# dillonalaird/pysvihmm

Hardware: AMD Instinct MI355X
Metric: obs-state updates/sec (T*K/s) per SVI E-step, K=64 Gaussian HMM (higher is better)
Workload: dtype f64

## Files before the change

include/svihmm_debug.h:

```cpp
#ifndef SVIHMM_DEBUG_H
#define SVIHMM_DEBUG_H

#include "svihmm.h"

#ifdef __cplusplus
extern "C" {
#endif

#define SVIHMM_NKERN 12
#define SVIHMM_PROF_SLOTS 0x40000000
int svihmm_profile_enable(svihmm_ctx* h, int32_t on);
int svihmm_profile_reset(svihmm_ctx* h);
int svihmm_profile_read(svihmm_ctx* h, double ms_out[SVIHMM_NKERN],
                        int64_t count_out[SVIHMM_NKERN]);
const char* svihmm_kernel_name(int32_t slot);
const char* svihmm_last_kernel_name(svihmm_ctx* h, int32_t slot);
#define SVIHMM_NVARIANT 24
enum {
  SVIHMM_VAR_SVI_LOOP = 0,
  SVIHMM_VAR_STATS = 1,
  SVIHMM_VAR_FB = 2,
  SVIHMM_VAR_EMISSION_MT = 3,
  SVIHMM_VAR_PIPELINE = 4,
  SVIHMM_VAR_EMISSION_ORBIT = 5,
  SVIHMM_VAR_CHAIN = 6,
  SVIHMM_VAR_SWEEP_FAMILY = 7,
  SVIHMM_VAR_STATS_CHUNKS = 8,
  SVIHMM_VAR_CENTRING = 9,
  SVIHMM_VAR_STATS_TILING = 10,
  SVIHMM_VAR_ALLREDUCE_COORDS = 11,
  SVIHMM_VAR_STATS_LDS3 = 12,
  SVIHMM_VAR_WIDE_SWEEPS = 13,
  SVIHMM_VAR_WIDE_TRAN_BLOCK = 14,
  SVIHMM_VAR_WIDE_POSTERIOR = 15,
  SVIHMM_VAR_RENORM4 = 16,
  SVIHMM_VAR_MSG_LAYOUT = 17
};
enum {
  SVIHMM_SVI_LOOP_EVENTS = 1,
  SVIHMM_SVI_LOOP_LOSE_CONCURRENCY = 2,
  SVIHMM_SVI_LOOP_STUCK_GATE = 3,
  SVIHMM_SVI_LOOP_NO_ELBO = 9,
  SVIHMM_STATS_DBUF = 2,
  SVIHMM_STATS_PIPELINED = 3,
  SVIHMM_FB_WAVE = 1,
  SVIHMM_FB_LOG_MFMA = 2,
  SVIHMM_FB_SCALED = 3,
  SVIHMM_EMISSION_MT_NT4 = 1,
  SVIHMM_PIPELINE_UNFUSED = 1,
  SVIHMM_PIPELINE_TWO_STREAM = 2,
  SVIHMM_PIPELINE_FUSED_ALL = 3,
  SVIHMM_PIPELINE_FUSED_EMISSION = 5,
  SVIHMM_PIPELINE_F32_OWN = 6,
  SVIHMM_EMISSION_ORBIT_OFF = 1,
  SVIHMM_EMISSION_ORBIT_128 = 2,
  SVIHMM_EMISSION_ORBIT_F64 = 3,
  SVIHMM_EMISSION_ORBIT_BF16_SMALL = 4,
  SVIHMM_EMISSION_ORBIT_64 = 5,
  SVIHMM_EMISSION_ORBIT_GENERIC_EDGES = 6,
  SVIHMM_EMISSION_ORBIT_128_GENERIC_EDGES = 7,
  SVIHMM_EMISSION_ORBIT_BF16_128 = 8,
  SVIHMM_CHAIN_OFF = 1,
  SVIHMM_SWEEP_FAMILY_ONE_TILE = 1,
  SVIHMM_SWEEP_FAMILY_TILES = 2,
  SVIHMM_SWEEP_FAMILY_WAVE_LIN = 3,
  SVIHMM_SWEEP_FAMILY_WAVE_LIN4 = 4,
  SVIHMM_SWEEP_FAMILY_SKIP = 9,
  SVIHMM_CENTRING_OFF = 1,
  SVIHMM_CENTRING_PULL_STARTS = 2,
  SVIHMM_STATS_TILING_FIVE = 1,
  SVIHMM_STATS_TILING_F32_MFMA = 2,
  SVIHMM_STATS_TILING_BF16_SMALL = 3,
  SVIHMM_ALLREDUCE_COORDS_ON = 1,
  SVIHMM_STATS_LDS3_OFF = 1,
  SVIHMM_STATS_LDS3_FLAT = 2,
  SVIHMM_WIDE_SWEEPS_16 = 1,
  SVIHMM_WIDE_SWEEPS_THETA_OLD = 2,
  SVIHMM_WIDE_SWEEPS_THETA_OWN_STEP = 3,
  SVIHMM_WIDE_TRAN_BLOCK_64 = 1,
  SVIHMM_WIDE_POSTERIOR_PASS = 1,
  SVIHMM_WIDE_POSTERIOR_PASS_ALL = 2,
  SVIHMM_RENORM4_OFF = 1,
  SVIHMM_MSG_LAYOUT_ROW_MAJOR = 1
};
int svihmm_set_variant(svihmm_ctx* h, int32_t which, int32_t value);
int svihmm_svi_recoveries(svihmm_ctx* h, int32_t* out);
// ... 9 lines not shown
```

pysvihmm_amd/_lib.py:

```python
import ctypes as C
import os

import numpy as np

_HERE = os.path.dirname(os.path.abspath(__file__))
LIB_PATH = os.path.join(_HERE, "libsvihmm_hip.so")

ABI_VERSION = 3
NKERN = 12
PROF_SLOTS = 0x40000000
MASK_AS_NAN = 1
TRANS_WRAP = 2
USE_HOST_LLIKS = 4
KEEP_LBETA = 8
SVI_KEEP_WINDOW = 16
SVI_MIN_PSEUDOCOUNT = 2.5e-3
LTRAN_LINEAR_MIN = -600.0
NIW_MAX_D = 96
DIAG_MAX_D = 128
MCAT_MAX_D = 128
MCAT_MAX_F = 1024
POISSON_MAX_D = 128
POISSON_MAX_COUNT = (1 << 20) - 1
PGAUSS_MAX_D = 128
PGAUSS_ABSENT = 1e150
LTRAN_F32_MIN = -60.0
F64, F32 = 0, 1
GROW_METHOD = {"auto": 0, "literal": 1, "products": 2}
VARIANT = {
    "svi_loop": 0, "stats": 1, "fb": 2, "emission_mt": 3, "pipeline": 4, "emission_orbit": 5, "chain": 6,
    "sweep_family": 7, "stats_chunks": 8, "centring": 9, "stats_tiling": 10, "allreduce_coords": 11,
    "stats_lds3": 12, "wide_sweeps": 13, "wide_tran_block": 14, "wide_posterior": 15, "renorm4": 16,
    "msg_layout": 17,
}
EMISSION_ORBIT_128 = 2
EMISSION_ORBIT_GENERIC_EDGES = 6
EMISSION_ORBIT_128_GENERIC_EDGES = 7

_lib = None

_c_double_p = C.POINTER(C.c_double)
_c_int64_p = C.POINTER(C.c_int64)
_c_uint8_p = C.POINTER(C.c_uint8)

SIGNATURES = {
    "svihmm_last_error": (C.c_char_p, []),
    "svihmm_abi_version": (C.c_int, []),
    "svihmm_device_count": (C.c_int, [C.POINTER(C.c_int)]),
    "svihmm_create": (C.c_int, [C.c_int, C.POINTER(C.c_void_p)]),
    "svihmm_destroy": (C.c_int, [C.c_void_p]),
    "svihmm_sync": (C.c_int, [C.c_void_p]),
    "svihmm_set_precision": (C.c_int, [C.c_void_p, C.c_int32]),
    "svihmm_get_precision": (C.c_int, [C.c_void_p, C.POINTER(C.c_int32), C.POINTER(C.c_int32)]),
    "svihmm_set_obs": (C.c_int, [C.c_void_p, _c_double_p, C.c_int64, C.c_int32, _c_uint8_p]),
    "svihmm_set_globals": (C.c_int, [C.c_void_p, C.c_int32, _c_double_p, _c_double_p]),
    "svihmm_set_emission_niw": (C.c_int, [C.c_void_p, C.c_int32, C.c_int32, _c_double_p,
                                          _c_double_p, _c_double_p, _c_double_p]),
    "svihmm_set_emission_diag": (C.c_int, [C.c_void_p, C.c_int32, C.c_int32, _c_double_p,
                                           _c_double_p, _c_double_p, _c_double_p]),
    "svihmm_set_lliks": (C.c_int, [C.c_void_p, _c_double_p, C.c_int32, C.c_int32]),
    "svihmm_loglik": (C.c_int, [C.c_void_p, _c_int64_p, C.c_int32, C.c_int32, C.c_uint32,
                                _c_double_p]),
    "svihmm_forward_backward": (C.c_int, [C.c_void_p, _c_int64_p, C.c_int32, C.c_int32,
                                          C.c_uint32, _c_double_p, _c_double_p, _c_double_p,
                                          _c_double_p]),
    "svihmm_packed_size": (C.c_int64, [C.c_int32, C.c_int32]),
    "svihmm_estep_minibatch": (C.c_int, [C.c_void_p, _c_int64_p, C.c_int32, C.c_int32,
                                         C.c_uint32, _c_double_p]),
    "svihmm_read_packed": (C.c_int, [C.c_void_p, _c_double_p]),
    "svihmm_suffstats": (C.c_int, [C.c_void_p, _c_int64_p, C.c_int32, C.c_int32, C.c_uint32,
# ... 159 lines not shown
```

pysvihmm_amd/csrc/host.h:

```cpp
#pragma once
#include <hip/hip_runtime.h>
#include <rccl/rccl.h>

#include <cmath>
#include <cstdint>
#include <cstdio>
#include <cstring>
#include <cstdlib>
#include <string>
#include <type_traits>
#include <vector>

#include "../../include/svihmm.h"
#include "../../include/svihmm_debug.h"
#include "svihmm_common.h"

extern thread_local std::string g_err;
inline int fail(const std::string& m) { g_err = m; return 1; }
#define HIPCK(x)                                                                   \
  do {                                                                             \
    hipError_t e_ = (x);                                                           \
    if (e_ != hipSuccess)                                                          \
      return fail(std::string(#x) + ": " + hipGetErrorString(e_) + " (" __FILE__ \
                  ":" + std::to_string(__LINE__) + ")");                           \
// ... 77 lines not shown
  int eK = 0, eD = 0, Kp = 0, F = 0, Fp = 0;
  Buf theta, theta_orb, fab, niw, cat_table, partc, prior, vlb_aux, gen_z;
  int64_t gen_T = 0;
  double* vlb_host = nullptr;
  int prior_K = 0, prior_D = 0, vlb_host_K = 0;
  void *slack_a = nullptr, *slack_t = nullptr;
  int slack_k = 0;
  void* orb_zero_p = nullptr; size_t orb_zero_n = 0;
  const double* chain_kbef = nullptr; int chain_C = 0, chain_L = 0, chain_T = 0;
  int lb_pending = 0;
  bool orb_valid = false;
  Buf uwb;
  void* uw_zero_p = nullptr;
  bool uw_valid = false;
  Buf uwd;
  void* uwd_zero_p = nullptr; size_t uwd_zero_n = 0;
  bool uwd_valid = false, emd_attr_set[2] = {false, false};
  bool emb_attr_set = false;
  EmisFamily fam = EF_NIW;
  int V = 0;
  Buf mcat_meta;
  int pois_C = 0; Buf pois_logfact; std::vector<double> pois_lf_host;
  Buf pg_origin;
  bool tab_diag = false;
  void* theta_zero_p = nullptr; size_t theta_zero_n = 0;
  int tabD = -1;
  struct PinSlot { void* p = nullptr; size_t cap = 0; hipEvent_t ev = nullptr; bool busy = false; };
  PinSlot pins[6];
  int pin_next = 0;
  struct StartSlot { void* p = nullptr; size_t cap = 0; int used_it = -1; };
  StartSlot svi_starts[8];
  const int64_t* starts_pending = nullptr;
  int starts_pending_n = 0;
  bool starts_sync_call = false, starts_slot_inflight = false;
  void* starts_slot = nullptr; size_t starts_slot_cap = 0;
  int svi_upload_it = -1;
  int* pin_status = nullptr;
  double* mirror = nullptr; size_t mirror_cap = 0;
  bool mirror_valid = false;
  bool status_pending = false;
  bool status_auto = false;
  bool have_emission = false;
  Buf starts, ll, la, lb, q, lse_part, local_lb, logz, part, packed, scratch;
  Buf user_q, user_starts;
  std::vector<int64_t> seq_off;
  Buf seq_off_d, seq_q, seq_work, seq_ord, seq_out;
  bool seq_internal = false;
  bool seq_result = false;
  Buf sub_obs, sub_mask, sub_tab;
  bool seq_subset = false;
  Buf labels, sub_labels;
  bool have_labels = false;
  int32_t label_max = -1; int64_t label_max_row = -1;
  Buf sets, sub_sets;
  bool have_sets = false;
  int32_t sets_K = 0, sets_W = 0;
  Buf dec_tab;
  std::vector<char> dec_host;
  int dec_result = 0;
  int post_kind = 0, post_K = 0, post_fam = -1;
  Buf heldout;
  Buf vit;
  Buf kexp, hx, gx, zfac, llE, m_ll, m_la, m_lb, chain, chain2;
  Buf ll0, a0v, a0e;
  bool lin_mode = false;
  bool q_valid = false;
// ... 162 lines not shown
int ensure_stats(svihmm_ctx* h, int64_t nchunk_total);
int flush_lb(svihmm_ctx* h, hipStream_t stream);
int launch_diag_to_theta(svihmm_ctx* h, int K, int D);
int launch_emission(svihmm_ctx* h, int B, int Lm, uint32_t flags, bool scaled = false, const int64_t* starts_dev = nullptr, double* out = nullptr, double* kexp_out = nullptr, hipStream_t stream = nullptr, size_t min_lds = 0, double* ll0_out = nullptr, bool clamp_labels = true);
int check_labels_fit(const svihmm_ctx* h);
int check_sets_fit(const svihmm_ctx* h);
int check_clamp_fit(const svihmm_ctx* h);
int launch_fb(svihmm_ctx* h, int B, int Lm, int dir0, int ndir, const double* ll = nullptr, double* la = nullptr, double* lb = nullptr);
int launch_fb_fused(svihmm_ctx* h, int B, int Lm, bool want_lb, bool total);
bool emission_row_tile_orbit(const svihmm_ctx* h, int64_t n);
bool step_major_ok(const svihmm_ctx* h, int B, int Lm, uint32_t flags, bool lin);
int launch_fb_lin(svihmm_ctx* h, int B, int Lm, bool total);
int launch_fb_lin_range(svihmm_ctx* h, int b0, int nb, int Lm, hipStream_t stream);
int launch_niw_to_theta(svihmm_ctx* h, int K, int D, double* logdet_out, const SviStepArgs* step = nullptr);
bool step_theta_ok(const svihmm_ctx* h, int K, int D);
int launch_posterior(svihmm_ctx* h, int B, int Lm, bool total);
int launch_scale_ll(svihmm_ctx* h, int B, int Lm);
int launch_scale_ll_f32(svihmm_ctx* h, int B, int Lm);
bool f32_wide_ok(const svihmm_ctx* h, int64_t n);
bool stats_bf16w_shape_ok(const svihmm_ctx* h, int64_t n);
int launch_stats(svihmm_ctx* h, int B, int Lq, int off, int Lm, uint32_t flags);
int launch_stats_finalize(svihmm_ctx* h, int64_t nchunk, hipStream_t stream);
int launch_stats_range(svihmm_ctx* h, int b0, int nb, int Lq, int off, int Lm, uint32_t flags, StatsPlan plan, int64_t chunk_base, hipStream_t stream,
                       const double* qsrc = nullptr, const int64_t* starts_src = nullptr);
int launch_stats_posteriors(svihmm_ctx* h, const double* q, const int64_t* starts_dev, int B, int Lm, uint32_t flags);
int launch_sum_lb(svihmm_ctx* h, int B, hipStream_t stream);
int materialise(svihmm_ctx* h, int b0, int nb);
int prepare_ll(svihmm_ctx* h, const int64_t* starts, int B, int Lm, uint32_t flags, bool need_obs_for_stats, bool lin = false);
StatsPlan stats_plan(const svihmm_ctx* h, int64_t n, int forced = 0);
int upload_feature_table(svihmm_ctx* h, int D, int K, bool diag = false);
bool use_chain(const svihmm_ctx* h, int B, int Lm);
int wait_globals(svihmm_ctx* h);
int svi_flush_elbo(svihmm_ctx* h);
int ensure_starts_pulled(svihmm_ctx* h);
int cat_uncentre(svihmm_ctx* h, int counts = -1);
extern "C++" inline std::string emission_d_message(const svihmm_ctx* h) {
  const FamTraits& t = FAM_TRAITS[h->fam];
  if (!t.columns) return "emission D does not match obs D";
  return std::string(t.setter) + ": the family has D = " + std::to_string(h->eD) + " " + t.columns +
         ", the resident observations have " + std::to_string(h->D);
}
int launch_fb_chain(svihmm_ctx* h, int Lm, bool total);
int launch_emission_deferred(svihmm_ctx* h);
int launch_viterbi(svihmm_ctx* h, int B, int Lm, const double* ll, bool want_z, int32_t** dz_out, double** dscore_out);
int launch_ffbs_windows(svihmm_ctx* h, const int64_t* starts, int B, int Lm, uint32_t flags, const double* logA, int S,
                        const double* uniforms, uint64_t seed, bool want_lalpha, int32_t** dz_out, const double** dla_out);
int launch_grow_products(svihmm_ctx* h, int n, int W, const double* ll, const int32_t* off, const int32_t* smax, int half0,
                         int m, int inc, double eps, int rule, int trace_cap, int32_t** half_out, int32_t** steps_out,
                         double** trace_out);
int launch_grow_state(svihmm_ctx* h, int n, int trace_cap, const int64_t* centers, const double* init);
int launch_grow_probe(svihmm_ctx* h, int n, int nact, const int32_t* idx, int b, int m, bool first, int inc, int cutoff,
                      double eps, int rule, int trace_cap, int32_t* active_host);
int grow_state_results(svihmm_ctx* h, int n, int trace_cap, const int32_t** ist_out, const double** trace_out);
bool sweep_emission_ok(const svihmm_ctx* h, int B, int Lq, int off, int Lm, uint32_t flags);
bool sweep_mixed_ok(const svihmm_ctx* h, int B, int Lq, int off, int Lm, uint32_t flags);
bool sweep_stats_ok(const svihmm_ctx* h, int B, int Lq, int off, int Lm, uint32_t flags);
int launch_sweep_stats(svihmm_ctx* h, int B, int Lq, int off, int Lm, uint32_t flags);
SviSync sweep_gate(svihmm_ctx* h, hipStream_t stream);
int launch_fb_sequences(svihmm_ctx* h, int nseq, const int32_t* order, const int64_t* seq_off, int64_t row_base,
                        int64_t span, int maxlen, const double* ll, double* q, double* seq_lb);
int launch_seq_finish(svihmm_ctx* h, int N, const int64_t* seq_off, bool wrap, const double* q, const double* seq_lb,
                      double* q0);
int launch_seq_gather(svihmm_ctx* h, int M, const int64_t* tab, int maxlen, double* obs_out, uint8_t* mask_out,
                      int32_t* labels_out, uint64_t* sets_out);
int64_t viterbi_sequences_chunks(const svihmm_ctx* h);
int launch_viterbi_sequences(svihmm_ctx* h, const double* ll, bool want_z, int32_t** dz_out, double** dscore_out);
int launch_ffbs_sequences(svihmm_ctx* h, uint32_t flags, const double* logA, int S, const double* uniforms, uint64_t seed,
// ... 5 lines not shown
```

pysvihmm_amd/csrc/kernels_recursion.h:

```cpp
#pragma once

template <int KMAX>
__global__ __launch_bounds__(64) void k_fb_wave(
    const double* __restrict__ ll, const double* __restrict__ Aexp,
    const double* __restrict__ mod_init, int Lm, int K, int dir0,
    double* __restrict__ la_out, double* __restrict__ lb_out) {
  __shared__ double p_s[2][KMAX];
  const int b = blockIdx.x, dir = dir0 + blockIdx.y, j = threadIdx.x;
  const bool valid = j < K;
  double a[KMAX];
#pragma unroll
  for (int i = 0; i < KMAX; ++i) {
    double v = 0.0;
    if (valid && i < K) v = (dir == 0) ? Aexp[i * K + j] : Aexp[j * K + i];
    a[i] = v;
  }
  const double* llb = ll + (size_t)b * Lm * K;
  const double NEG_INF = -INFINITY;
  int cur = 0;
  if (dir == 0) {
    double* out = la_out + (size_t)b * Lm * K;
    double la = valid ? mod_init[j] + llb[j] : NEG_INF;
    if (valid) out[j] = la;
    double llnext = (valid && Lm > 1) ? llb[K + j] : 0.0;
// ... 569 lines not shown
  __device__ __forceinline__ void init(int bfirst, int B, int wstride, int K, bool shared_rows, bool smaj = false) {
    lane = threadIdx.x & 63; wave = threadIdx.x >> 6;
    li = lane & 15; lg = lane >> 4;
    j = wave * 16 + li;
    vj = FULL || (j < K);
    jc = vj ? j : 0;
    b0 = bfirst;
#pragma unroll
    for (int r = 0; r < 4; ++r) {
      const int gw = b0 + LV<CT>::crow(lg, r);
      gwc[r] = gw < B ? gw : B - 1;
      oR[r] = shared_rows ? 0u : (unsigned)(gwc[r] - b0) * (unsigned)wstride;
      oE[r] = (smaj ? (unsigned)(gwc[r] - b0) : oR[r]) * (unsigned)K + (unsigned)jc;
    }
    tsK = smaj ? (size_t)msg_group_windows(B, b0) * K : (size_t)K;
    const int gww = b0 + LV<CT>::crow(lg, wave & 3);
    oRw = shared_rows ? 0u : (unsigned)((gww < B ? gww : B - 1) - b0) * (unsigned)wstride;
  }
};
__device__ __forceinline__ double sel4(const double (&v)[4], int w) {
  return w == 0 ? v[0] : (w == 1 ? v[1] : (w == 2 ? v[2] : v[3]));
}

struct LinChain {
  const double* init_vec;
  const double* init_exp;
  const double* term_vec;
  const double* term_exp;
  const double* kbefore;
  double* Mout;
  double* MoutT;
  double* Mh;
  int smaj;
};

template <int MODE, bool BS, typename ST>
struct LinCT { typedef typename std::conditional<std::is_same<ST, float>::value && MODE == 0 && !BS, float, double>::type t; };
template <int NW, bool FULL, int MODE, bool BS = false, typename ST = double>
__device__ __forceinline__ void fwd_lin_body(
    LinShared<NW, typename LinCT<MODE, BS, ST>::t>& sh, const ST* __restrict__ Eh, const double* __restrict__ kexp,
    const double* __restrict__ Aexp, const double* __restrict__ a0v,
    const double* __restrict__ a0e, int B, int Lm,
    int wstride, int K, ST* __restrict__ ah, double* __restrict__ hx,
    double* __restrict__ local_lb, double* __restrict__ logz, double2* __restrict__ zfac,
    const LinChain& ch) {
  constexpr int KS = 4 * NW;
  typedef typename LinCT<MODE, BS, ST>::t CT;
  typedef typename LV<CT>::v4 cv4;
  LinLane<NW, FULL, CT> L;
  const int chunk = MODE == 2 ? blockIdx.x / NW : 0, rgrp = MODE == 2 ? blockIdx.x % NW : 0;
  constexpr bool SMOK = NW == 4 && FULL && MODE == 0 && !BS && std::is_same<ST, double>::value;
  L.init(MODE == 2 ? chunk : blockIdx.x * 16, MODE == 2 ? chunk + 1 : B, wstride, K, MODE == 2, SMOK && ch.smaj);
  const size_t tsK = SMOK ? L.tsK : (size_t)K;
  const int li = L.li, lg = L.lg, j = L.j, jc = L.jc, wave = L.wave;
  const bool vj = L.vj;
  CT Bv[BS ? 1 : KS];
  if (!BS) {
#pragma unroll
    for (int kk = 0; kk < KS; ++kk) {
      const int k = lin_kslot<NW>(lg, kk);
      Bv[BS ? 0 : kk] = (k < K && vj) ? (CT)Aexp[(size_t)k * K + jc] : (CT)0;
    }
  }
  const double* __restrict__ Bcol = Aexp + jc;
  const size_t wrow = (size_t)L.b0 * wstride;
  const ST* __restrict__ Eb = Eh + wrow * K;
  ST* __restrict__ ab = ah + wrow * K;
  double* __restrict__ hb = hx + wrow;
  const int i1 = Lm > 1 ? 1 : 0, i2 = Lm > 2 ? 2 : i1;
  double h[4], mant[4], hsum[4];
  CT ea[4], eb[4];
  int ex[4];
  {
    CT a0[4];
    if (MODE == 0) {
#pragma unroll
      for (int r = 0; r < 4; ++r) {
        a0[r] = vj ? (CT)a0v[(size_t)L.gwc[r] * K + jc] : (CT)0;
        h[r] = a0e[L.gwc[r]];
      }
    } else if (MODE == 1) {
#pragma unroll
      for (int r = 0; r < 4; ++r) {
        a0[r] = vj ? (CT)ch.init_vec[(size_t)L.gwc[r] * K + jc] : (CT)0;
        h[r] = ch.init_exp[L.gwc[r]];
      }
    } else {
#pragma unroll
      for (int r = 0; r < 4; ++r) { a0[r] = (vj && j == rgrp * 16 + LV<CT>::crow(lg, r)) ? (CT)1 : (CT)0; h[r] = 0.0; }
    }
#pragma unroll
    for (int r = 0; r < 4; ++r) ea[r] = (Eb + (size_t)i1 * tsK)[L.oE[r]];
#pragma unroll
    for (int r = 0; r < 4; ++r) eb[r] = (Eb + (size_t)i2 * tsK)[L.oE[r]];
#pragma unroll
    for (int r = 0; r < 4; ++r) {
      if (MODE != 2) {
        if (NW % 4 != 0) hb[L.oR[r]] = h[r];
        if (FULL || vj) ab[L.oE[r]] = a0[r];
      }
      sh.P[0][LV<CT>::crow(lg, r)][j] = a0[r];
      mant[r] = 1.0; ex[r] = 0; hsum[r] = 0.0;
    }
    if (MODE != 2 && NW % 4 == 0) hb[L.oRw] = sel4(h, wave & 3);
  }
  __syncthreads();
  auto step = [&](const int t, auto curc, CT (&er)[4]) {
    constexpr int CUR = decltype(curc)::value, NXT = 1 - CUR;
// ... 1468 lines not shown
```

pysvihmm_amd/csrc/svihmm_hip.hip:

```cpp
#include "host.h"
#include <algorithm>
#include "device_helpers.h"
#include "kernels_misc.h"
#include "kernels_heldout.h"
#include "kernels_expect.h"
#include "kernels_svi.h"

thread_local std::string g_err;
static const char* kKernNames[SVIHMM_NKERN] = {
    "emission", "forward_backward", "posterior", "stats", "finalize", "ffbs_sample",
    "misc", "allreduce", "h2d", "d2h", "reserved0", "reserved1"};

extern "C" {

const char* svihmm_last_error(void) { return g_err.c_str(); }
int svihmm_abi_version(void) { return SVIHMM_ABI_VERSION; }
const char* svihmm_kernel_name(int32_t slot) {
  return (slot >= 0 && slot < SVIHMM_NKERN) ? kKernNames[slot] : "";
}

int svihmm_device_count(int* n_out) {
  int n = 0;
  hipError_t e = hipGetDeviceCount(&n);
  if (e != hipSuccess) { *n_out = 0; return fail(std::string("hipGetDeviceCount: ") + hipGetErrorString(e)); }
// ... 840 lines not shown
                  std::to_string(starts[b] + Lm - 1) + ") holds rows of two sequences: sequence " + std::to_string(s) +
                  " ends at row " + std::to_string(so[s + 1] - 1) + " (svihmm_set_sequences)");
  }
  return 0;
}
static int check_windows(svihmm_ctx* h, const int64_t* starts, int B, int Lm, bool need_obs) {
  if (B <= 0 || Lm <= 0) return fail("bad window batch (B, Lm must be positive)");
  if (need_obs) {
    if (h->T <= 0) return fail("no observations: call svihmm_set_obs first");
    if (!starts) return fail("starts is NULL");
    for (int b = 0; b < B; ++b)
      if (starts[b] < 0 || starts[b] + Lm > h->T)
        return fail("window " + std::to_string(b) + " out of range");
    CK(check_window_sequences(h, "", starts, B, Lm));
  }
  return 0;
}

static int pull_small(svihmm_ctx* h, void* dst, const void* pin, size_t bytes) {
  const size_t n = bytes / 8;
  unsigned blocks = (unsigned)((n + 1023) / 1024);
  if (blocks > 512) blocks = 512;
  if (blocks < 1) blocks = 1;
  void* dpin = nullptr;
  HIPCK(hipHostGetDevicePointer(&dpin, const_cast<void*>(pin), 0));
  hipLaunchKernelGGL(k_pull, dim3(blocks), dim3(256), 0, h->stream, (const unsigned long long*)dpin,
                     (unsigned long long*)dst, n);
  HIPCK(hipGetLastError());
  return 0;
}

int ensure_starts_pulled(svihmm_ctx* h) {
  if (!h->starts_pending) return 0;
  void* dst = h->starts.p;
  const int64_t* src = h->starts_pending;
  h->starts_pending = nullptr;
  hipLaunchKernelGGL(k_pull, dim3(1), dim3(256), 0, h->stream, (const unsigned long long*)src,
                     (unsigned long long*)dst, (size_t)h->starts_pending_n);
  HIPCK(hipGetLastError());
  return 0;
}
static int upload_starts(svihmm_ctx* h, const int64_t* starts, int B) {
  CK(ensure(h->starts, (size_t)B * sizeof(int64_t)));
  h->starts_pending = nullptr;
  const size_t nb = (size_t)B * sizeof(int64_t);
  if (h->svi_upload_it >= 0 && nb <= (size_t)1 << 20) {
    svihmm_ctx::StartSlot& ss = h->svi_starts[h->svi_upload_it % 8];
    if (ss.used_it >= 0 && h->svi_flags && h->svi_ts && 2 * ss.used_it + 1 < h->svi_ts_cap) {
      volatile unsigned long long* ts = &h->svi_ts[2 * ss.used_it + 1];
      int spins = 0;
      while (*ts == 0 && ++spins < 200000) { for (volatile int w = 0; w < 50; ++w) {} }
      if (*ts == 0) HIPCK(hipStreamSynchronize(h->stream));
    } else if (ss.used_it >= 0 && 2 * ss.used_it + 1 < (int)h->svi_ev.size())
      HIPCK(hipEventSynchronize(h->svi_ev[2 * ss.used_it + 1]));
    if (nb > ss.cap) {
      if (ss.p) hipHostFree(ss.p);
      ss.p = nullptr; ss.cap = 0;
      HIPCK(hipHostMalloc(&ss.p, nb + 4096, hipHostMallocMapped));
      ss.cap = nb + 4096;
    }
    std::memcpy(ss.p, starts, nb);
    void* dpin = nullptr;
    HIPCK(hipHostGetDevicePointer(&dpin, ss.p, 0));
    h->starts_pending = (const int64_t*)dpin; h->starts_pending_n = B;
    ss.used_it = h->svi_upload_it;
  } else if (h->starts_sync_call && nb <= (size_t)1 << 20) {
    if (h->starts_slot_inflight) { HIPCK(hipStreamSynchronize(h->stream)); h->starts_slot_inflight = false; }
    if (nb > h->starts_slot_cap) {
      if (h->starts_slot) hipHostFree(h->starts_slot);
      h->starts_slot = nullptr; h->starts_slot_cap = 0;
      HIPCK(hipHostMalloc(&h->starts_slot, nb + 4096, hipHostMallocMapped));
      h->starts_slot_cap = nb + 4096;
    }
    std::memcpy(h->starts_slot, starts, nb);
    void* dpin = nullptr;
    HIPCK(hipHostGetDevicePointer(&dpin, h->starts_slot, 0));
    h->starts_pending = (const int64_t*)dpin; h->starts_pending_n = B;
    h->starts_slot_inflight = true;
  } else if (nb <= (size_t)4 << 20) {
    void* pin = nullptr;
    int slot = 0;
    CK(pinned(h, nb, &pin, &slot));
    std::memcpy(pin, starts, nb);
    CK(pull_small(h, h->starts.p, pin, nb));
    CK(pin_release(h, slot));
  } else {
    HIPCK(hipMemcpyAsync(h->starts.p, starts, nb, hipMemcpyHostToDevice, h->stream));
  }
  return 0;
}



static int pick_fb(const svihmm_ctx* h, int B, int Lm, bool want_logs) {
  int var = h->variant[SVIHMM_VAR_FB];
  if (h->K > 256 || h->exact_log) return SVIHMM_FB_WAVE;
  if (h->K > 64) {
    if (var == SVIHMM_FB_LOG_MFMA) var = SVIHMM_FB_WAVE;
    if (var == 0) var = (use_chain(h, B, Lm) || (B >= cu_scaled(h, 192) && !want_logs)) ? SVIHMM_FB_SCALED : SVIHMM_FB_WAVE;
    if (var == SVIHMM_FB_SCALED && !use_chain(h, B, Lm) && (size_t)16 * Lm * h->K * sizeof(double) >= ((size_t)1 << 32))
      var = SVIHMM_FB_WAVE;
    return var;
  }
  if (var == 0)
    var = want_logs ? (use_chain(h, B, Lm) ? SVIHMM_FB_SCALED : B >= cu_scaled(h, 192) ? SVIHMM_FB_LOG_MFMA : SVIHMM_FB_WAVE)
                    : SVIHMM_FB_SCALED;
  if (var == SVIHMM_FB_SCALED && !use_chain(h, B, Lm) &&
      !(B < lin_wave_max(h) && h->variant[SVIHMM_VAR_SWEEP_FAMILY] != SVIHMM_SWEEP_FAMILY_TILES) &&
      (size_t)16 * Lm * h->K * sizeof(double) >= ((size_t)1 << 32))
    var = SVIHMM_FB_LOG_MFMA;
  return var;
}

int wait_globals(svihmm_ctx* h) {
  if (h->globals_ev) {
    HIPCK(hipStreamWaitEvent(h->stream, h->globals_ev, 0));
    h->globals_ev = nullptr;
  }
  return 0;
}
// ... 2382 lines not shown
```

pysvihmm_amd/csrc/tu_emission.hip:

```cpp
#include "host.h"
#include "device_helpers.h"
#include "kernels_emission.h"
#define SVIHMM_MCAT_EMISSION
#include "kernels_mcat.h"
#define SVIHMM_POISSON_EMISSION
#include "kernels_poisson.h"
#define SVIHMM_PGAUSS_EMISSION
#include "kernels_pgauss.h"
#define SVIHMM_LABELS_CLAMP
#include "kernels_labels.h"

template <class Kern, class... Args>
static void launch_lookup_columns(svihmm_ctx* h, hipStream_t stream, int64_t n, Kern staged, Kern through_l2, bool tlds,
                                  int rb, size_t tb, size_t ib, Args... args) {
  int64_t rpw = (n + 8 * (int64_t)h->ncu - 1) / (8 * (int64_t)h->ncu);
  rpw = std::max<int64_t>(tlds ? 256 : rb, (rpw + rb - 1) / rb * rb);
  if (rpw > 1 << 20) rpw = 1 << 20;
  const size_t lds = (tlds ? tb : 0) + ib;
  const dim3 grid((unsigned)((n + rpw - 1) / rpw));
  if (tlds) {
    hipFuncSetAttribute((const void*)staged, hipFuncAttributeMaxDynamicSharedMemorySize, (int)lds);
    hipLaunchKernelGGL(staged, grid, dim3(256), lds, stream, args..., (int)rpw);
  } else {
    hipLaunchKernelGGL(through_l2, grid, dim3(256), lds, stream, args..., (int)rpw);
// ... 254 lines not shown
      (n >= 8192 || h->variant[SVIHMM_VAR_EMISSION_ORBIT] == SVIHMM_EMISSION_ORBIT_BF16_SMALL)) {
    uint4* uwp = nullptr;
    const int64_t* pend = nullptr;
    int pend_n = 0;
    if (own_starts && h->starts_pending && h->starts_pending_n == B && stream == h->stream) {
      pend = h->starts_pending; pend_n = B; h->starts_pending = nullptr;
      starts_dev = pend;
    } else CK(device_starts());
    CK(emb_buffers(h, &uwp));
    if (!h->uw_valid) {
      const double* dmu = (const double*)h->niw.p;
      const double* dsg = dmu + (size_t)K * D;
      const double* dka = dsg + (size_t)K * D * D;
      const double* dnu = dka + K;
#define NIWU(DM) hipLaunchKernelGGL(k_niw_to_theta_wave<DM>, dim3(K), dim3(64), 0, stream, dmu, dsg, dka, dnu, K, D, Kp, \
                                    (double*)nullptr, (int*)nullptr, (double*)nullptr, (double*)nullptr, uwp)
      if (D <= 8) NIWU(8); else if (D <= 16) NIWU(16); else NIWU(32);
#undef NIWU
      HIPCK(hipGetLastError());
      h->uw_valid = true;
    }
    const int MTe = (n + 255) / 256 >= 256 ? 2 : 1;
    const size_t lds = (size_t)EMB_REC + (size_t)4 * (32 * MTe) * 64 * 4;
    if (!h->emb_attr_set) {
      HIPCK(hipFuncSetAttribute((const void*)k_emission_bf16x3<2>, hipFuncAttributeMaxDynamicSharedMemorySize,
                                (int)((size_t)EMB_REC + (size_t)4 * 64 * 64 * 4)));
      HIPCK(hipFuncSetAttribute((const void*)k_emission_bf16x3<1>, hipFuncAttributeMaxDynamicSharedMemorySize,
                                (int)((size_t)EMB_REC + (size_t)4 * 32 * 64 * 4)));
      h->emb_attr_set = true;
    }
    if (MTe == 2)
      hipLaunchKernelGGL(k_emission_bf16x3<2>, dim3((unsigned)((n + 255) / 256)), dim3(256), lds, stream,
                         (const double*)h->obs.p, mk, starts_dev, n, Lm, D, K, (const char*)uwp,
                         flags, (float*)out, kexp_out, ll0_out, pend ? (int64_t*)h->starts.p : (int64_t*)nullptr, pend_n);
    else if (h->variant[SVIHMM_VAR_EMISSION_ORBIT] == SVIHMM_EMISSION_ORBIT_BF16_128)
      hipLaunchKernelGGL(k_emission_bf16x3<1>, dim3((unsigned)((n + 127) / 128)), dim3(256), lds, stream,
                         (const double*)h->obs.p, mk, starts_dev, n, Lm, D, K, (const char*)uwp,
                         flags, (float*)out, kexp_out, ll0_out, pend ? (int64_t*)h->starts.p : (int64_t*)nullptr, pend_n);
    else {
#define EMH(NHV, RWV) hipLaunchKernelGGL((k_emission_bf16x3h<NHV, RWV>), dim3((unsigned)((n + 32 * RWV - 1) / (32 * RWV))), \
                         dim3(64 * (NHV) * (RWV)), (size_t)(NHV) * EMB_REC + (size_t)(RWV) * 32 * 64 * 4, stream,      \
                         (const double*)h->obs.p, mk, starts_dev, n, Lm, D, K, (const char*)uwp,                       \
                         flags, (float*)out, kexp_out, ll0_out, pend ? (int64_t*)h->starts.p : (int64_t*)nullptr, pend_n)
      if ((n + 31) / 32 <= 520) EMH(4, 1); else EMH(2, 2);
#undef EMH
    }
    HIPCK(hipGetLastError());
    return 0;
  }
  const bool wide32 = !scaled && h->cur_f32 && K > 64;
  if (h->fam != EF_DIAG && ((scaled && (flags & SVIHMM_INT_ST32) && K <= 64) || wide32) && emd_shape_ok(K, D) && h->niw.p &&
      h->variant[SVIHMM_VAR_EMISSION_ORBIT] != SVIHMM_EMISSION_ORBIT_F64 && min_lds == 0 && bf16_batch_floor_ok(h, n)) {
    uint4* uwp = nullptr;
    CK(device_starts());
    CK(emd_buffers(h, K, &uwp));
    if (!h->uwd_valid) {
      const double* dmu = (const double*)h->niw.p;
      const double* dsg = dmu + (size_t)K * D;
      const double* dka = dsg + (size_t)K * D * D;
      const double* dnu = dka + K;
      hipLaunchKernelGGL(k_niw_to_theta_wave<64>, dim3(K), dim3(64), 0, stream, dmu, dsg, dka, dnu, K, D, Kp,
                         (double*)nullptr, (int*)nullptr, (double*)nullptr, (double*)nullptr, uwp);
      HIPCK(hipGetLastError());
      h->uwd_valid = true;
    }
    const size_t lds = (size_t)2 * EMD_REC + (size_t)8 * 32 * 64 * 4;
    const int wi = wide32 ? 1 : 0;
    if (!h->emd_attr_set[wi]) {
      if (wide32) HIPCK(hipFuncSetAttribute((const void*)k_emission_bf16x3d<true>, hipFuncAttributeMaxDynamicSharedMemorySize, (int)lds));
      else HIPCK(hipFuncSetAttribute((const void*)k_emission_bf16x3d<false>, hipFuncAttributeMaxDynamicSharedMemorySize, (int)lds));
      h->emd_attr_set[wi] = true;
    }
    dim3 grid((unsigned)((n + 255) / 256), wide32 ? (unsigned)((K + 63) / 64) : 1u);
    if (wide32)
      hipLaunchKernelGGL(k_emission_bf16x3d<true>, grid, dim3(512), lds, stream, (const double*)h->obs.p, mk, starts_dev, n, Lm,
                         D, K, (const char*)uwp, flags, (float*)out, kexp_out, ll0_out);
    else
      hipLaunchKernelGGL(k_emission_bf16x3d<false>, grid, dim3(512), lds, stream, (const double*)h->obs.p, mk, starts_dev, n, Lm,
                         D, K, (const char*)uwp, flags, (float*)out, kexp_out, ll0_out);
    HIPCK(hipGetLastError());
    return 0;
  }
  int var = 2;
  if (h->fam != EF_DIAG && scaled && K <= 64 && D >= 8 && D <= 40 && D % 8 == 0 &&
      h->variant[SVIHMM_VAR_EMISSION_ORBIT] != SVIHMM_EMISSION_ORBIT_OFF && min_lds == 0) {
    const int NT = Kp / 16, LEN = D + D / 2 + 1;
    const int nks = (D / 4) * (D / 2 + 1) + (D / 2 + 1 + 3) / 4;
    const int64_t* pend = nullptr;
    int pend_n = 0;
    if (own_starts && h->starts_pending && h->starts_pending_n == B && stream == h->stream) {
      pend = h->starts_pending; pend_n = B; h->starts_pending = nullptr;
      starts_dev = pend;
    } else CK(device_starts());
    if (!h->orb_valid) {
      CK(ensure(h->theta_orb, (size_t)nks * 4 * Kp * sizeof(double)));
      hipLaunchKernelGGL(k_theta_orbit, dim3(nks * 4), dim3(64), 0, stream, (const double*)h->theta.p,
                         D, Kp, NT, (double*)h->theta_orb.p);
      HIPCK(hipGetLastError());
      h->orb_valid = true;
    }
    if ((n + 127) / 128 < h->ncu && !orbit_128(h) &&
        h->variant[SVIHMM_VAR_EMISSION_ORBIT] != SVIHMM_EMISSION_ORBIT_64) {
      const int R0 = 3 * NT * 256 > 16 * LEN + 1 ? 3 * NT * 256 : ((16 * LEN + 1) & ~1);
      const size_t lds = (size_t)(R0 + 16 * NT + 16) * 8 + 16;
      dim3 grid((unsigned)((n + 15) / 16));
      if (h->em_defer_req && NT == 4 && stream == h->stream && out == (double*)h->ll.p && !(flags & SVIHMM_INT_ST32)) {
        h->em_def.active = true;
        h->em_def.starts = starts_dev; h->em_def.starts_copy = pend ? (int64_t*)h->starts.p : nullptr; h->em_def.nstarts = pend_n;
        h->em_def.B = B; h->em_def.Lm = Lm; h->em_def.flags = flags;
        h->em_def.out = out; h->em_def.kexp = kexp_out; h->em_def.ll0 = ll0_out;
        return 0;
      }
#define EMK(NTV) hipLaunchKernelGGL((k_emission_orbit_ks<NTV>), grid, dim3(256), lds, stream,                      \
                                    (const double*)h->obs.p, mk, starts_dev, n, Lm, D, K,                          \
                                    (const double*)h->theta_orb.p, flags, out, kexp_out, ll0_out,                  \
                                    pend ? (int64_t*)h->starts.p : (int64_t*)nullptr, pend_n)
      if (NT == 4) EMK(4); else if (NT == 3) EMK(3); else if (NT == 2) EMK(2); else EMK(1);
#undef EMK
      HIPCK(hipGetLastError());
      return 0;
    }
    const int MTo = ((n + 127) / 128 < h->ncu && !orbit_128(h)) ? 1 : 2;
    const int rows = 64 * MTo;
    const int smB = (h->step_major && own_out && own_starts) ? B : 0;
    const size_t lds = (size_t)rows * LEN * 8 + rows * 9 + ((MTo == 2 && D == 32) ? 1024 : 0);
    dim3 grid((unsigned)((n + rows - 1) / rows));
    const int lean = K == Kp && !(flags & SVIHMM_INT_ST32) &&
                     h->variant[SVIHMM_VAR_EMISSION_ORBIT] != SVIHMM_EMISSION_ORBIT_GENERIC_EDGES &&
                     h->variant[SVIHMM_VAR_EMISSION_ORBIT] != SVIHMM_EMISSION_ORBIT_128_GENERIC_EDGES &&
                     (int64_t)h->T * D * 8 < ((int64_t)1 << 32) &&
                     ((int64_t)32 * Lm + rows) * K * 8 < ((int64_t)1 << 32);
#define EMO(NTV, UV, MTV) hipLaunchKernelGGL((k_emission_orbit<NTV, UV, MTV>), grid, dim3(256), lds, stream,  \
                                        (const double*)h->obs.p, mk, starts_dev, n, Lm, D, K,               \
                                        (const double*)h->theta_orb.p, flags, out, kexp_out, ll0_out,               \
                                        pend ? (int64_t*)h->starts.p : (int64_t*)nullptr, pend_n, smB, lean)
#define EMOM(NTV, UV) do { if (MTo == 1) EMO(NTV, UV, 1); else EMO(NTV, UV, 2); } while (0)
    if (D % 16 == 0) { if (NT == 4) EMOM(4, 4); else if (NT == 3) EMOM(3, 4); else if (NT == 2) EMOM(2, 4); else EMOM(1, 4); }
    else             { if (NT == 4) EMOM(4, 2); else if (NT == 3) EMOM(3, 2); else if (NT == 2) EMOM(2, 2); else EMOM(1, 2); }
#undef EMOM
#undef EMO
    HIPCK(hipGetLastError());
    return 0;
  }
  CK(device_starts());
  if (var == 2) {
    const int DS = (D + 2) | 1;
    int MT = h->variant[SVIHMM_VAR_EMISSION_MT] > 0 ? h->variant[SVIHMM_VAR_EMISSION_MT] : 2;
    if (MT != 2 && MT != 4) MT = 2;
    size_t lds = (size_t)(64 * MT) * DS * 8 + (size_t)h->Fp * 4 + (size_t)(64 * MT) * 9;
    if (lds > 150 * 1024 && MT == 4) { MT = 2; lds = (size_t)128 * DS * 8 + (size_t)h->Fp * 4 + 128 * 9; }
    if (lds < min_lds) lds = min_lds;
    if (lds > 150 * 1024 && scaled) return fail("emission: D too large for the scaled sweeps");
    if (lds > 150 * 1024 && h->fam == EF_DIAG) return fail("emission: D too large for the diagonal family's kernel");
    if (lds > 150 * 1024) return fail("emission: D too large for the LDS-staged GEMM kernel");
    {
      const int ntile = Kp / 16;
      int NT = (ntile % 4 == 0) ? 4 : (ntile % 2 == 0) ? 2 : 1;
      if (!scaled && MT == 2 && ntile % 8 == 0 && h->variant[SVIHMM_VAR_EMISSION_MT] != SVIHMM_EMISSION_MT_NT4) NT = 8;
      if (scaled) { NT = ntile; MT = 2; }
      const int rows = 64 * MT;
      dim3 grid((unsigned)((n + rows - 1) / rows), ntile / NT);
#define EMM_LAUNCH(NTV, MTV, SC)                                                             \
  do {                                                                                        \
    if (lds > 64 * 1024)                                                                      \
      hipFuncSetAttribute((const void*)k_emission_mfma<NTV, MTV, SC>,                         \
                          hipFuncAttributeMaxDynamicSharedMemorySize, (int)lds);              \
    hipLaunchKernelGGL((k_emission_mfma<NTV, MTV, SC>), grid, dim3(256), lds, stream,         \
                       (const double*)h->obs.p, mk, starts_dev, n, Lm, D, K,                  \
// ... 86 lines not shown
```

pysvihmm_amd/csrc/tu_recursion.hip:

```cpp
#include <algorithm>
#include "host.h"
#include "device_helpers.h"
#include "kernels_ffbs_draw.h"
#include "kernels_recursion.h"
#include "kernels_viterbi.h"
#include "kernels_ffbs_windows.h"
#include "kernels_grow.h"
#include "kernels_sequences.h"
#include "kernels_decode_sequences.h"
#define SVIHMM_LABELS_GATHER
#include "kernels_labels.h"

template <bool LDSBT, class Units>
static void vit_sweep(svihmm_ctx* h, unsigned n, size_t lds, const double* ll, const Units& units, unsigned char* psi,
                      int32_t* z, int32_t* zlast, double* score) {
  const int K = h->K;
  const double* lt = (const double*)h->ltran.p;
  const double* mi = (const double*)h->mod_init.p;
#define VITW(KM)                                                                                                   \
  hipLaunchKernelGGL((k_vit_wave<KM, LDSBT, Units>), dim3(n), dim3(64), lds, h->stream, ll, lt, mi, units, K, psi, \
                     z, zlast, score)
  if (K <= 16) VITW(16); else if (K <= 32) VITW(32); else if (K <= 64) VITW(64);
  else
    hipLaunchKernelGGL((k_vit_wide<LDSBT, Units>), dim3(n), dim3(256), lds, h->stream, ll, lt, mi, units, K, psi, z,
// ... 223 lines not shown
  do {                                                                                                        \
    const size_t lds = (size_t)(WT) * sizeof(LinShared<16>);                                                  \
    dim3 g2((unsigned)((nb + 16 * (WT) - 1) / (16 * (WT))), 2);                                               \
    hipFuncSetAttribute((const void*)k_sweeps_lin2<8, F, WT, float, true>, hipFuncAttributeMaxDynamicSharedMemorySize, (int)lds); \
    hipLaunchKernelGGL((k_sweeps_lin2<8, F, WT, float, true>), g2, dim3(512), lds, stream, Ef, kx,            \
                       (const float*)h->AexpF.p, (const float*)h->AexpTF.p, a0v, a0e, nb, Lm, K, af, bf, hx, gx, llb, lz, zf); \
  } while (0)
      if (w32) { if (K == 256) SWP2F(true, 2); else SWP2F(false, 2); }
      else if (K == 256) SWP2F(true, 1); else SWP2F(false, 1);
#undef SWP2F
      HIPCK(hipGetLastError());
      return 0;
    }
    if (nb < lin_wave_max(h) && h->variant[SVIHMM_VAR_SWEEP_FAMILY] != SVIHMM_SWEEP_FAMILY_TILES) {
      dim3 gw((unsigned)nb, 2);
#define WLF(KM, FK) hipLaunchKernelGGL((k_wave_lin<KM, FK, float>), gw, dim3(64), 0, stream, Ef, kx, (const double*)h->Aexp.p, \
                                       (const double*)h->AexpT.p, mi, l0, l0s, Lm, K, af, bf, hx,   \
                                       gx, llb, lz, zf)
#define WL4F(KM) hipLaunchKernelGGL((k_wave_lin4<KM, float>), gw, dim3(256), 0, stream, Ef, kx, (const double*)h->Aexp.p, \
                                    (const double*)h->AexpT.p, mi, l0, l0s, Lm, K, af, bf, hx, gx, \
                                    llb, lz, zf, gsy)
      if (wave_kernel && nb <= lin_waver_max(h) && Lm <= (1 << 20) &&
          h->variant[SVIHMM_VAR_SWEEP_FAMILY] != SVIHMM_SWEEP_FAMILY_WAVE_LIN4) {
        const SviSync gsy = sweep_gate(h, stream);
        hipLaunchKernelGGL((k_wave_linr<float, double>), gw, dim3(64), 0, stream, Ef, kx, (const double*)h->Aexp.p,
                           (const double*)h->AexpT.p, mi, l0, l0s, Lm, K, af, bf, hx, gx, llb, lz, zf, gsy);
      }
      else if (wave_kernel) { const SviSync gsy = sweep_gate(h, stream); WL4F(64); }
      else if (K <= 16) WLF(16, false); else if (K <= 32) WLF(32, false);
      else if (K == 64) WLF(64, true); else WLF(64, false);
#undef WLF
#undef WL4F
    } else {
      CK(launch_lin_init(h, b0, nb, Lm, stream));
      const LinChain none = {};
#define SWF(NWV, F) hipLaunchKernelGGL((k_sweeps_lin<NWV, F, 0, false, float>), grid, dim3(64 * NWV),              \
                                       sizeof(LinShared<NWV>), stream, Ef, kx, (const double*)h->Aexp.p,         \
                                       (const double*)h->AexpT.p, a0v, a0e, nb, Lm, Lm, K,   \
                                       af, bf, hx, gx, llb, lz, zf, none)
      if (NW == 1) { if (full) SWF(1, true); else SWF(1, false); }
      else if (NW == 2) { if (full) SWF(2, true); else SWF(2, false); }
      else if (NW == 3) { if (full) SWF(3, true); else SWF(3, false); }
      else { if (full) SWF(4, true); else SWF(4, false); }
#undef SWF
    }
    HIPCK(hipGetLastError());
    return 0;
  }
  if (K <= 64 && nb < lin_wave_max(h) && h->variant[SVIHMM_VAR_SWEEP_FAMILY] != SVIHMM_SWEEP_FAMILY_TILES) {
    dim3 gw((unsigned)nb, 2);
#define WL(KM, FK) hipLaunchKernelGGL((k_wave_lin<KM, FK>), gw, dim3(64), 0, stream, Eh, kx, (const double*)h->Aexp.p, \
                                      (const double*)h->AexpT.p, mi, l0, l0s, Lm, K, ah, bh, hx,  \
                                      gx, llb, lz, zf)
    if (wave_kernel) {
      const SviSync gsy = sweep_gate(h, stream);
      if (h->f32_ok && h->variant[SVIHMM_VAR_RENORM4] != SVIHMM_RENORM4_OFF)
        hipLaunchKernelGGL((k_wave_linr<double, double, 4>), gw, dim3(64), 0, stream, Eh, kx, (const double*)h->Aexp.p,
                           (const double*)h->AexpT.p, mi, l0, l0s, Lm, K, ah, bh, hx, gx, llb, lz, zf, gsy);
      else
        hipLaunchKernelGGL((k_wave_linr<double>), gw, dim3(64), 0, stream, Eh, kx, (const double*)h->Aexp.p,
                           (const double*)h->AexpT.p, mi, l0, l0s, Lm, K, ah, bh, hx, gx, llb, lz, zf, gsy);
    }
    else if (K <= 16) WL(16, false); else if (K <= 32) WL(32, false);
    else if (K == 64) WL(64, true); else WL(64, false);
#undef WL
    HIPCK(hipGetLastError());
    return 0;
  }
  CK(launch_lin_init(h, b0, nb, Lm, stream));
  LinChain none = {};
  if (h->step_major) {
    if (!(NW == 4 && full && b0 == 0 && nb == h->curB)) return fail("internal: step-major messages without their sweep kernel");
    none.smaj = 1;
  }
#define SWPX(NWV, F, BSV)                                                                                  \
  do {                                                                                                     \
    const size_t lds = sizeof(LinShared<NWV>);                                                             \
    if (lds > 64 * 1024)                                                                                   \
      hipFuncSetAttribute((const void*)k_sweeps_lin<NWV, F, 0, BSV>,                                       \
                          hipFuncAttributeMaxDynamicSharedMemorySize, (int)lds);                           \
    hipLaunchKernelGGL((k_sweeps_lin<NWV, F, 0, BSV>), grid, dim3(64 * NWV), lds, stream, Eh, kx,          \
                       (const double*)h->Aexp.p, (const double*)h->AexpT.p,                                \
                       a0v, a0e, nb, Lm, Lm, K, ah, bh, hx, gx, llb, lz, zf, none);    \
  } while (0)
#define SWP(NWV, F) SWPX(NWV, F, false)
  if (NW == 1) { if (full) SWP(1, true); else SWP(1, false); }
  else if (NW == 2) { if (full) SWP(2, true); else SWP(2, false); }
  else if (NW == 3) { if (full) SWP(3, true); else SWP(3, false); }
  else if (NW == 4) { if (full) SWP(4, true); else SWP(4, false); }
  else if (NW <= 8) { if (K == 128) SWPX(8, true, true); else SWPX(8, false, true); }
  else {
#define SWP2(F, WT)                                                                                        \
  do {                                                                                                     \
    const size_t lds = (size_t)(WT) * sizeof(LinShared<16>);                                               \
    dim3 g2((unsigned)((nb + 16 * (WT) - 1) / (16 * (WT))), 2);                                            \
    hipFuncSetAttribute((const void*)k_sweeps_lin2<8, F, WT>, hipFuncAttributeMaxDynamicSharedMemorySize,  \
                        (int)lds);                                                                         \
    hipLaunchKernelGGL((k_sweeps_lin2<8, F, WT>), g2, dim3(512), lds, stream, Eh, kx,                      \
                       (const double*)h->Aexp.p, (const double*)h->AexpT.p, a0v, a0e,  \
                       nb, Lm, K, ah, bh, hx, gx, llb, lz, zf);                                            \
  } while (0)
    const bool w32 = 2 * ((nb + 15) / 16) > h->ncu && h->variant[SVIHMM_VAR_WIDE_SWEEPS] != SVIHMM_WIDE_SWEEPS_16;
    if (NW <= 12 && h->variant[SVIHMM_VAR_SWEEP_FAMILY] != SVIHMM_SWEEP_FAMILY_TILES) {
// ... 880 lines not shown
```

Before: 21.23 billion.

## Fold linear-init into sweep kernel and skip redundant starts uploads

Removes the separate lin_init kernel launch by computing the initial scaled alpha (mod_init + l0, max-reduced per row via DPP and LDS, then exponentiated with a power-of-two shift) inside k_sweeps_lin. Also caches the host copy of sequence starts and skips the pinned upload when the same starts are passed again, invalidating the cache wherever a kernel writes the device starts buffer. Both aim to cut per-step launch and small-transfer overhead. The cost is an extra __syncthreads and reduction at sweep start, a host memcmp, and added complexity in keeping the cache valid.

```diff
diff --git a/include/svihmm_debug.h b/include/svihmm_debug.h
--- a/include/svihmm_debug.h
+++ b/include/svihmm_debug.h
@@ -52,6 +52,7 @@
   SVIHMM_PIPELINE_FUSED_ALL = 3,
   SVIHMM_PIPELINE_FUSED_EMISSION = 5,
   SVIHMM_PIPELINE_F32_OWN = 6,
+  SVIHMM_PIPELINE_UNFOLDED = 7,
   SVIHMM_EMISSION_ORBIT_OFF = 1,
   SVIHMM_EMISSION_ORBIT_128 = 2,
   SVIHMM_EMISSION_ORBIT_F64 = 3,
diff --git a/pysvihmm_amd/_lib.py b/pysvihmm_amd/_lib.py
--- a/pysvihmm_amd/_lib.py
+++ b/pysvihmm_amd/_lib.py
@@ -36,6 +36,7 @@
 EMISSION_ORBIT_128 = 2
 EMISSION_ORBIT_GENERIC_EDGES = 6
 EMISSION_ORBIT_128_GENERIC_EDGES = 7
+PIPELINE_UNFOLDED = 7
 
 _lib = None
 
diff --git a/pysvihmm_amd/csrc/host.h b/pysvihmm_amd/csrc/host.h
--- a/pysvihmm_amd/csrc/host.h
+++ b/pysvihmm_amd/csrc/host.h
@@ -133,6 +133,8 @@
   StartSlot svi_starts[8];
   const int64_t* starts_pending = nullptr;
   int starts_pending_n = 0;
+  std::vector<int64_t> starts_host;
+  bool starts_known = false;
   bool starts_sync_call = false, starts_slot_inflight = false;
   void* starts_slot = nullptr; size_t starts_slot_cap = 0;
   int svi_upload_it = -1;
@@ -361,7 +363,18 @@
 bool use_chain(const svihmm_ctx* h, int B, int Lm);
 int wait_globals(svihmm_ctx* h);
 int svi_flush_elbo(svihmm_ctx* h);
+enum { FOLD_STARTS = 2, FOLD_LIN_INIT = 4 };
+#ifndef SVIHMM_AB_UNFOLD
+#define SVIHMM_AB_UNFOLD 0
+#endif
+inline bool fold_on(const svihmm_ctx* h, int which) {
+  return !(SVIHMM_AB_UNFOLD & which) && h->variant[SVIHMM_VAR_PIPELINE] != SVIHMM_PIPELINE_UNFOLDED;
+}
 int ensure_starts_pulled(svihmm_ctx* h);
+inline int64_t* starts_write_ptr(svihmm_ctx* h) {
+  h->starts_known = false;
+  return (int64_t*)h->starts.p;
+}
 int cat_uncentre(svihmm_ctx* h, int counts = -1);
 extern "C++" inline std::string emission_d_message(const svihmm_ctx* h) {
   const FamTraits& t = FAM_TRAITS[h->fam];
diff --git a/pysvihmm_amd/csrc/kernels_recursion.h b/pysvihmm_amd/csrc/kernels_recursion.h
--- a/pysvihmm_amd/csrc/kernels_recursion.h
+++ b/pysvihmm_amd/csrc/kernels_recursion.h
@@ -625,6 +625,9 @@
   double* MoutT;
   double* Mh;
   int smaj;
+  const double* mod_init;
+  const double* l0;
+  size_t l0s;
 };
 
 template <int MODE, bool BS, typename ST>
@@ -666,7 +669,35 @@
   int ex[4];
   {
     CT a0[4];
-    if (MODE == 0) {
+    if (MODE == 0 && !BS && ch.mod_init) {
+      double v[4], m[4];
+      const double mi = vj ? ch.mod_init[jc] : 0.0;
+#pragma unroll
+      for (int r = 0; r < 4; ++r) {
+        v[r] = vj ? mi + ch.l0[(size_t)L.gwc[r] * ch.l0s + jc] : -INFINITY;
+        m[r] = v[r];
+        m[r] = fmax(m[r], dpp_mov_f64<0xB1>(m[r]));
+        m[r] = fmax(m[r], dpp_mov_f64<0x4E>(m[r]));
+        m[r] = fmax(m[r], dpp_mov_f64<0x141>(m[r]));
+        m[r] = fmax(m[r], dpp_mov_f64<0x140>(m[r]));
+      }
+      double* mx = reinterpret_cast<double*>(&sh.P[1][0][0]);
+      if (li == 0) {
+#pragma unroll
+        for (int r = 0; r < 4; ++r) mx[wave * 16 + LV<CT>::crow(lg, r)] = m[r];
+      }
+      __syncthreads();
+      const double* __restrict__ kbw = kexp + wrow;
+#pragma unroll
+      for (int r = 0; r < 4; ++r) {
+        double mw = -INFINITY;
+#pragma unroll
+        for (int w = 0; w < NW; ++w) mw = fmax(mw, mx[w * 16 + LV<CT>::crow(lg, r)]);
+        const double H = (mw > -1e300 && mw < 1e300) ? ceil(mw * LOG2E_D) : 0.0;
+        a0[r] = vj ? (CT)exp(fma(-H, LN2_LO_D, fma(-H, LN2_HI_D, v[r]))) : (CT)0;
+        h[r] = H - kbw[L.oR[r]];
+      }
+    } else if (MODE == 0) {
 #pragma unroll
       for (int r = 0; r < 4; ++r) {
         a0[r] = vj ? (CT)a0v[(size_t)L.gwc[r] * K + jc] : (CT)0;
diff --git a/pysvihmm_amd/csrc/svihmm_hip.hip b/pysvihmm_amd/csrc/svihmm_hip.hip
--- a/pysvihmm_amd/csrc/svihmm_hip.hip
+++ b/pysvihmm_amd/csrc/svihmm_hip.hip
@@ -896,7 +896,7 @@
 
 int ensure_starts_pulled(svihmm_ctx* h) {
   if (!h->starts_pending) return 0;
-  void* dst = h->starts.p;
+  void* dst = starts_write_ptr(h);
   const int64_t* src = h->starts_pending;
   h->starts_pending = nullptr;
   hipLaunchKernelGGL(k_pull, dim3(1), dim3(256), 0, h->stream, (const unsigned long long*)src,
@@ -905,6 +905,7 @@
   return 0;
 }
 static int upload_starts(svihmm_ctx* h, const int64_t* starts, int B) {
+  if (!h->starts.p || (size_t)B * sizeof(int64_t) > h->starts.cap) h->starts_known = false;
   CK(ensure(h->starts, (size_t)B * sizeof(int64_t)));
   h->starts_pending = nullptr;
   const size_t nb = (size_t)B * sizeof(int64_t);
@@ -927,6 +928,7 @@
     void* dpin = nullptr;
     HIPCK(hipHostGetDevicePointer(&dpin, ss.p, 0));
     h->starts_pending = (const int64_t*)dpin; h->starts_pending_n = B;
+    h->starts_known = false;
     ss.used_it = h->svi_upload_it;
   } else if (h->starts_sync_call && nb <= (size_t)1 << 20) {
     if (h->starts_slot_inflight) { HIPCK(hipStreamSynchronize(h->stream)); h->starts_slot_inflight = false; }
@@ -940,16 +942,22 @@
     void* dpin = nullptr;
     HIPCK(hipHostGetDevicePointer(&dpin, h->starts_slot, 0));
     h->starts_pending = (const int64_t*)dpin; h->starts_pending_n = B;
+    h->starts_known = false;
     h->starts_slot_inflight = true;
   } else if (nb <= (size_t)4 << 20) {
+    if (h->starts_known && h->starts_host.size() == (size_t)B && std::memcmp(h->starts_host.data(), starts, nb) == 0 &&
+        fold_on(h, FOLD_STARTS))
+      return 0;
     void* pin = nullptr;
     int slot = 0;
     CK(pinned(h, nb, &pin, &slot));
     std::memcpy(pin, starts, nb);
-    CK(pull_small(h, h->starts.p, pin, nb));
+    CK(pull_small(h, starts_write_ptr(h), pin, nb));
     CK(pin_release(h, slot));
+    h->starts_host.assign(starts, starts + B);
+    h->starts_known = true;
   } else {
-    HIPCK(hipMemcpyAsync(h->starts.p, starts, nb, hipMemcpyHostToDevice, h->stream));
+    HIPCK(hipMemcpyAsync(starts_write_ptr(h), starts, nb, hipMemcpyHostToDevice, h->stream));
   }
   return 0;
 }
diff --git a/pysvihmm_amd/csrc/tu_emission.hip b/pysvihmm_amd/csrc/tu_emission.hip
--- a/pysvihmm_amd/csrc/tu_emission.hip
+++ b/pysvihmm_amd/csrc/tu_emission.hip
@@ -310,16 +310,16 @@
     if (MTe == 2)
       hipLaunchKernelGGL(k_emission_bf16x3<2>, dim3((unsigned)((n + 255) / 256)), dim3(256), lds, stream,
                          (const double*)h->obs.p, mk, starts_dev, n, Lm, D, K, (const char*)uwp,
-                         flags, (float*)out, kexp_out, ll0_out, pend ? (int64_t*)h->starts.p : (int64_t*)nullptr, pend_n);
+                         flags, (float*)out, kexp_out, ll0_out, pend ? starts_write_ptr(h) : (int64_t*)nullptr, pend_n);
     else if (h->variant[SVIHMM_VAR_EMISSION_ORBIT] == SVIHMM_EMISSION_ORBIT_BF16_128)
       hipLaunchKernelGGL(k_emission_bf16x3<1>, dim3((unsigned)((n + 127) / 128)), dim3(256), lds, stream,
                          (const double*)h->obs.p, mk, starts_dev, n, Lm, D, K, (const char*)uwp,
-                         flags, (float*)out, kexp_out, ll0_out, pend ? (int64_t*)h->starts.p : (int64_t*)nullptr, pend_n);
+                         flags, (float*)out, kexp_out, ll0_out, pend ? starts_write_ptr(h) : (int64_t*)nullptr, pend_n);
     else {
 #define EMH(NHV, RWV) hipLaunchKernelGGL((k_emission_bf16x3h<NHV, RWV>), dim3((unsigned)((n + 32 * RWV - 1) / (32 * RWV))), \
                          dim3(64 * (NHV) * (RWV)), (size_t)(NHV) * EMB_REC + (size_t)(RWV) * 32 * 64 * 4, stream,      \
                          (const double*)h->obs.p, mk, starts_dev, n, Lm, D, K, (const char*)uwp,                       \
-                         flags, (float*)out, kexp_out, ll0_out, pend ? (int64_t*)h->starts.p : (int64_t*)nullptr, pend_n)
+                         flags, (float*)out, kexp_out, ll0_out, pend ? starts_write_ptr(h) : (int64_t*)nullptr, pend_n)
       if ((n + 31) / 32 <= 520) EMH(4, 1); else EMH(2, 2);
 #undef EMH
     }
@@ -384,7 +384,7 @@
       dim3 grid((unsigned)((n + 15) / 16));
       if (h->em_defer_req && NT == 4 && stream == h->stream && out == (double*)h->ll.p && !(flags & SVIHMM_INT_ST32)) {
         h->em_def.active = true;
-        h->em_def.starts = starts_dev; h->em_def.starts_copy = pend ? (int64_t*)h->starts.p : nullptr; h->em_def.nstarts = pend_n;
+        h->em_def.starts = starts_dev; h->em_def.starts_copy = pend ? starts_write_ptr(h) : nullptr; h->em_def.nstarts = pend_n;
         h->em_def.B = B; h->em_def.Lm = Lm; h->em_def.flags = flags;
         h->em_def.out = out; h->em_def.kexp = kexp_out; h->em_def.ll0 = ll0_out;
         return 0;
@@ -392,7 +392,7 @@
 #define EMK(NTV) hipLaunchKernelGGL((k_emission_orbit_ks<NTV>), grid, dim3(256), lds, stream,                      \
                                     (const double*)h->obs.p, mk, starts_dev, n, Lm, D, K,                          \
                                     (const double*)h->theta_orb.p, flags, out, kexp_out, ll0_out,                  \
-                                    pend ? (int64_t*)h->starts.p : (int64_t*)nullptr, pend_n)
+                                    pend ? starts_write_ptr(h) : (int64_t*)nullptr, pend_n)
       if (NT == 4) EMK(4); else if (NT == 3) EMK(3); else if (NT == 2) EMK(2); else EMK(1);
 #undef EMK
       HIPCK(hipGetLastError());
@@ -411,7 +411,7 @@
 #define EMO(NTV, UV, MTV) hipLaunchKernelGGL((k_emission_orbit<NTV, UV, MTV>), grid, dim3(256), lds, stream,  \
                                         (const double*)h->obs.p, mk, starts_dev, n, Lm, D, K,               \
                                         (const double*)h->theta_orb.p, flags, out, kexp_out, ll0_out,               \
-                                        pend ? (int64_t*)h->starts.p : (int64_t*)nullptr, pend_n, smB, lean)
+                                        pend ? starts_write_ptr(h) : (int64_t*)nullptr, pend_n, smB, lean)
 #define EMOM(NTV, UV) do { if (MTo == 1) EMO(NTV, UV, 1); else EMO(NTV, UV, 2); } while (0)
     if (D % 16 == 0) { if (NT == 4) EMOM(4, 4); else if (NT == 3) EMOM(3, 4); else if (NT == 2) EMOM(2, 4); else EMOM(1, 4); }
     else             { if (NT == 4) EMOM(4, 2); else if (NT == 3) EMOM(3, 2); else if (NT == 2) EMOM(2, 2); else EMOM(1, 2); }
diff --git a/pysvihmm_amd/csrc/tu_recursion.hip b/pysvihmm_amd/csrc/tu_recursion.hip
--- a/pysvihmm_amd/csrc/tu_recursion.hip
+++ b/pysvihmm_amd/csrc/tu_recursion.hip
@@ -279,8 +279,9 @@
 #undef WLF
 #undef WL4F
     } else {
-      CK(launch_lin_init(h, b0, nb, Lm, stream));
-      const LinChain none = {};
+      LinChain none = {};
+      if (fold_on(h, FOLD_LIN_INIT)) { none.mod_init = mi; none.l0 = l0; none.l0s = l0s; }
+      else CK(launch_lin_init(h, b0, nb, Lm, stream));
 #define SWF(NWV, F) hipLaunchKernelGGL((k_sweeps_lin<NWV, F, 0, false, float>), grid, dim3(64 * NWV),              \
                                        sizeof(LinShared<NWV>), stream, Ef, kx, (const double*)h->Aexp.p,         \
                                        (const double*)h->AexpT.p, a0v, a0e, nb, Lm, Lm, K,   \
@@ -314,8 +315,9 @@
     HIPCK(hipGetLastError());
     return 0;
   }
-  CK(launch_lin_init(h, b0, nb, Lm, stream));
   LinChain none = {};
+  if (NW <= 4 && fold_on(h, FOLD_LIN_INIT)) { none.mod_init = mi; none.l0 = l0; none.l0s = l0s; }
+  else CK(launch_lin_init(h, b0, nb, Lm, stream));
   if (h->step_major) {
     if (!(NW == 4 && full && b0 == 0 && nb == h->curB)) return fail("internal: step-major messages without their sweep kernel");
     none.smaj = 1;
```

Result: no change. 21.26 billion (median of 2 runs) (+0.1%).
